# luisayang-malaxiangguo/Hybrid-GMRES

Hardware: AMD Instinct MI355X
Metric: GMRES iters/sec + SpMV GB/s (% HBM roofline), 2-D phantom A, 1/2/4/8 GPU (higher is better)
Workload: dtype f64

## Files before the change

hybrid-gmres_amd/csrc/capi.cpp:

```cpp
#include <limits.h>
#include <link.h>
#include <sched.h>

#include <chrono>
#include <cmath>
#include <cstdio>
#include <cstdlib>
#include <algorithm>
#include <cstring>
#include <set>
#include <vector>

#include "internal.h"

namespace hgm {

void DevBuf::ensure(size_t b) {
    if (b <= bytes) return;
    release();
    if (hipMalloc(&p, b) != hipSuccess) {
        p = nullptr;
        bytes = 0;
        throw Error{HGM_E_NOMEM, "hipMalloc failed for workspace (" + std::to_string(b) + " bytes)"};
    }
// ... 394 lines not shown

HGM_API void hgm_ctx_destroy(hgm_ctx* c) {
    if (!c) return;
    (void)hipSetDevice(c->device);
    if (c->stream) (void)hipStreamSynchronize(c->stream);
    if (c->host_stats)
        std::fprintf(stderr, "hgm host stats: %ld pipeline waits, %.3f ms blocked (%.2f us/wait)\n", c->waits,
                     c->wait_s * 1e3, c->waits ? c->wait_s * 1e6 / c->waits : 0.0);
    if (c->nccl) ncclCommDestroy(c->nccl);
    c->timing.clear();
    for (auto e : c->timing.pool) (void)hipEventDestroy(e);
    c->ws.clear();
    if (c->dscal) (void)hipFree(c->dscal);
    if (c->hscal) (void)hipHostFree(c->hscal);
    if (c->hstage) (void)hipHostFree(c->hstage);
    if (c->hup) (void)hipHostFree(c->hup);
    if (c->hring) (void)hipHostFree(c->hring);
    if (c->ev_pipe) (void)hipEventDestroy(c->ev_pipe);
    for (auto e : c->ev_step)
        if (e) (void)hipEventDestroy(e);
    if (c->aux) {
        (void)hipStreamSynchronize(c->aux);
        (void)hipStreamDestroy(c->aux);
    }
    if (c->stream) (void)hipStreamDestroy(c->stream);
    delete c;
}

HGM_API const char* hgm_last_error(const hgm_ctx* c) { return c ? c->err.c_str() : "null context"; }

HGM_API int hgm_ctx_set_option(hgm_ctx* c, int option, double v) {
    if (!c) return HGM_E_ARG;
    hgm::Numerics& n = c->num;
    const bool b01 = v == 0.0 || v == 1.0;
    auto bad = [&](const char* what) {
        c->err = std::string("hgm_ctx_set_option: ") + what;
        return HGM_E_ARG;
    };
    if (!HGM_EXPERIMENTS) {
        bool variant = false;
        switch (option) {
            case HGM_OPT_FUSED_REGION: variant = v != 64; break;
            case HGM_OPT_FUSED_BS: variant = v != 1024; break;
            case HGM_OPT_FUSED_DBG: variant = v != 0; break;
            case HGM_OPT_FUSED_PF: variant = v != 2; break;
            case HGM_OPT_FUSED_KIND: variant = v != 1; break;
            case HGM_OPT_FUSED_WAVES: variant = v != 4; break;
            case HGM_OPT_FUSED_GROUP: variant = v != 8; break;
            case HGM_OPT_FUSED_DEPTH: variant = v != 2; break;
            case HGM_OPT_FUSED_PAIRS: variant = v != 1; break;
            case HGM_OPT_FUSED_ACC32: variant = v != 1; break;
            case HGM_OPT_FUSED_REDUCE: variant = !(v == 0 || v == 1); break;
            case HGM_OPT_FUSED_ROWPAIR: variant = !(v == 0 || v == 4); break;
            default: break;
        }
        if (variant) return bad("a measured variant of the one-pass kernel: experiments build only (HGM_EXPERIMENTS=1)");
    }
    switch (option) {
        case HGM_OPT_PARITY: if (!b01) return bad("parity is 0 or 1"); n.parity = v != 0; break;
        case HGM_OPT_MGS_FORM: if (!b01) return bad("mgs form is 0 or 1"); n.mgs_form = (int)v; break;
        case HGM_OPT_MGS_SINGLE: if (!b01) return bad("mgs single is 0 or 1"); n.mgs_single = v != 0; break;
        case HGM_OPT_GRAM_ERR: if (!b01) return bad("gram err is 0 or 1"); n.gram_err = v != 0; break;
        case HGM_OPT_GRAM_ERR_MIN: if (!(v >= 0.0)) return bad("gram err min >= 0"); n.gram_err_min = v; break;
        case HGM_OPT_RING_POLL: if (!b01) return bad("ring poll is 0 or 1"); n.ring_poll = v != 0; break;
        case HGM_OPT_PEND_NORM:
            if (!(v == 0.0 || v == 1.0 || v == 2.0)) return bad("pend norm is 0, 1 or 2");
            n.pend_norm = (int)v;
            break;
        case HGM_OPT_RECON_SERIAL:
            if (v != -1.0 && !b01) return bad("recon serial is -1, 0 or 1");
            n.recon_serial = (int)v;
            break;
        case HGM_OPT_RECON_SERIAL_N: if (!(v >= 0.0)) return bad("recon serial n >= 0"); n.recon_serial_n = (int64_t)v; break;
        case HGM_OPT_PIPE_DEPTH:
            if (!(v >= 1.0 && v <= 6.0) || v != (double)(int)v) return bad("pipe depth is 1..6");
            n.pipe_depth = (int)v;
            break;
        case HGM_OPT_SYNC_EVENT_FENCE: if (!b01) return bad("sync event fence is 0 or 1"); n.sync_event_fence = v != 0; break;
        case HGM_OPT_MGS_PPL:
            if (!(v >= 1.0 && v <= 8.0) || v != (double)(int)v) return bad("mgs ppl is 1..8");
            n.mgs_ppl = (int)v;
            break;
        case HGM_OPT_MGS1_PPL:
            if (!(v == 0.0 || v == 1.0 || v == 2.0 || v == 4.0)) return bad("mgs1 ppl is 0, 1, 2 or 4");
            n.mgs1_ppl = (int)v;
            break;
        case HGM_OPT_MGS_FUSED: n.mgs_fused = v != 0.0; break;
        case HGM_OPT_LSQR_DEV: n.lsqr_dev = v != 0.0; break;
        case HGM_OPT_PAGED16: n.paged16 = v != 0.0; break;
        case HGM_OPT_BAND_DUAL: n.band_dual = v != 0.0; break;
        case HGM_OPT_FUSED_AB: if (!b01) return bad("fused_ab is 0 or 1"); n.fused_ab = v != 0; break;
        case HGM_OPT_FUSED_REGION:
            if (!(v >= 8 && v <= 1024 && v == std::floor(v))) return bad("fused_region is an integer in [8, 1024]");
            n.fused_region = (int)v;
            break;
        case HGM_OPT_FUSED_BS:
            if (!(v == 512 || v == 1024)) return bad("fused_bs is 512 or 1024");
            n.fused_bs = (int)v;
            break;
        case HGM_OPT_FUSED_PF: if (v < 0 || v > 4) return bad("fused_pf is 0..4"); n.fused_pf = v < 1 ? 1 : (int)v; break;
        case HGM_OPT_KRYLOV_PAD: if (v < -1 || v > 65536 || v != (double)(int64_t)v || (v > 0 && (int64_t)v % 64)) return bad("krylov_pad is -1 or a multiple of 64 in 0..65536"); n.krylov_pad = (int)v; break;
        case HGM_OPT_FUSED_DBG:
            if (!(v >= 0 && v <= 15 && v == std::floor(v))) return bad("fused_dbg is 0..15");
            n.fused_dbg = (int)v;
            break;
        case HGM_OPT_FUSED_KIND: if (!b01) return bad("fused_kind is 0 or 1"); n.fused_kind = (int)v; break;
        case HGM_OPT_FUSED_WREGION:
            if (!(v >= 4 && v <= 256 && v == std::floor(v))) return bad("fused_wregion is an integer in [4, 256]");
            n.fused_wregion = (int)v;
            break;
        case HGM_OPT_FUSED_WAVES:
            if (!(v == 1 || v == 2 || v == 4)) return bad("fused_waves is 1, 2 or 4");
            n.fused_waves = (int)v;
            break;
        case HGM_OPT_FUSED_GROUP:
            if (!(v == 4 || v == 8)) return bad("fused_group is 4 or 8");
            n.fused_group = (int)v;
            break;
        case HGM_OPT_FUSED_DEPTH:
            if (!(v == 2 || v == 3 || v == 4)) return bad("fused_depth is 2, 3 or 4");
            n.fused_depth = (int)v;
            break;
        case HGM_OPT_FUSED_PAIRS: if (!b01) return bad("fused_pairs is 0 or 1"); n.fused_pairs = v != 0; break;
        case HGM_OPT_FUSED_ACC32:
            if (!(v == 0 || v == 1 || v == 2)) return bad("fused_acc32 is 0, 1 or 2");
            n.fused_acc32 = (int)v;
            break;
        case HGM_OPT_FUSED_PLAN_DEV: if (!b01) return bad("fused_plan_dev is 0 or 1"); n.fused_plan_dev = v != 0; break;
        case HGM_OPT_FUSED_REDUCE:
            if (!(v == 0 || v == 1 || v == 2 || v == 3 || v == 4)) return bad("fused_reduce is 0 to 4");
            n.fused_reduce = (int)v;
            break;
        case HGM_OPT_FUSED_ROWPAIR:
            if (!(v == 0 || v == 1 || v == 2 || v == 3 || v == 4)) return bad("fused_rowpair is 0 to 4");
            n.fused_rowpair = (int)v;
            break;
        case HGM_OPT_FUSED_VSTREAM:
            if (!(v == 0 || v == 1 || v == 2 || v == 3)) return bad("fused_vstream is 0 to 3");
            n.fused_vstream = (int)v;
            break;
        case HGM_OPT_LSQR_RES_IMG: if (!b01) return bad("lsqr_res_img is 0 or 1"); n.lsqr_res_img = v != 0; break;
        case HGM_OPT_LSMR_FUSE_NMON: if (!b01) return bad("lsmr_fuse_nmon is 0 or 1"); n.lsmr_fuse_nmon = v != 0; break;
        case HGM_OPT_HOST_SPIN_US:
            if (!(v == std::floor(v) && std::fabs(v) <= 1e9)) return bad("host_spin_us is an integer");
            g_host_spin_us.store((int)v);
            break;
        default: return bad("unknown option");
    }
    return HGM_OK;
}

HGM_API int hgm_ctx_get_option(const hgm_ctx* c, int option, double* v) {
    if (!c || !v) return HGM_E_ARG;
    const hgm::Numerics& n = c->num;
    switch (option) {
        case HGM_OPT_PARITY: *v = n.parity; break;
        case HGM_OPT_MGS_FORM: *v = n.mgs_form; break;
        case HGM_OPT_MGS_SINGLE: *v = n.mgs_single; break;
        case HGM_OPT_GRAM_ERR: *v = n.gram_err; break;
        case HGM_OPT_GRAM_ERR_MIN: *v = n.gram_err_min; break;
        case HGM_OPT_RING_POLL: *v = n.ring_poll; break;
        case HGM_OPT_PEND_NORM: *v = n.pend_norm; break;
        case HGM_OPT_RECON_SERIAL: *v = n.recon_serial; break;
        case HGM_OPT_RECON_SERIAL_N: *v = (double)n.recon_serial_n; break;
        case HGM_OPT_PIPE_DEPTH: *v = n.pipe_depth; break;
        case HGM_OPT_SYNC_EVENT_FENCE: *v = n.sync_event_fence; break;
        case HGM_OPT_MGS_PPL: *v = n.mgs_ppl; break;
        case HGM_OPT_MGS1_PPL: *v = n.mgs1_ppl; break;
        case HGM_OPT_MGS_FUSED: *v = n.mgs_fused; break;
        case HGM_OPT_LSQR_DEV: *v = n.lsqr_dev; break;
        case HGM_OPT_PAGED16: *v = n.paged16; break;
        case HGM_OPT_BAND_DUAL: *v = n.band_dual; break;
        case HGM_OPT_FUSED_AB: *v = n.fused_ab; break;
        case HGM_OPT_FUSED_REGION: *v = n.fused_region; break;
        case HGM_OPT_FUSED_BS: *v = n.fused_bs; break;
        case HGM_OPT_FUSED_DBG: *v = n.fused_dbg; break;
        case HGM_OPT_FUSED_PF: *v = n.fused_pf; break;
        case HGM_OPT_KRYLOV_PAD: *v = n.krylov_pad; break;
        case HGM_OPT_FUSED_KIND: *v = n.fused_kind; break;
        case HGM_OPT_FUSED_WREGION: *v = n.fused_wregion; break;
        case HGM_OPT_FUSED_WAVES: *v = n.fused_waves; break;
        case HGM_OPT_FUSED_GROUP: *v = n.fused_group; break;
        case HGM_OPT_FUSED_DEPTH: *v = n.fused_depth; break;
        case HGM_OPT_FUSED_PAIRS: *v = n.fused_pairs; break;
        case HGM_OPT_FUSED_ACC32: *v = n.fused_acc32; break;
        case HGM_OPT_FUSED_PLAN_DEV: *v = n.fused_plan_dev; break;
        case HGM_OPT_FUSED_REDUCE: *v = n.fused_reduce; break;
        case HGM_OPT_FUSED_ROWPAIR: *v = n.fused_rowpair; break;
        case HGM_OPT_FUSED_VSTREAM: *v = n.fused_vstream; break;
        case HGM_OPT_LSQR_RES_IMG: *v = n.lsqr_res_img; break;
        case HGM_OPT_LSMR_FUSE_NMON: *v = n.lsmr_fuse_nmon; break;
        case HGM_OPT_HOST_SPIN_US: *v = g_host_spin_us.load(); break;
        default: return HGM_E_ARG;
    }
    return HGM_OK;
}

HGM_API int hgm_ctx_synchronize(hgm_ctx* c) {
    if (!c) return HGM_E_ARG;
    HGM_TRY(c, sync(c));
    return HGM_OK;
}

HGM_API void* hgm_ctx_stream(hgm_ctx* c) { return c ? (void*)c->stream : nullptr; }

HGM_API int hgm_ctx_rank(const hgm_ctx* c, int* rank, int* world) {
    if (!c) return HGM_E_ARG;
    if (rank) *rank = c->rank;
    if (world) *world = c->world;
    return HGM_OK;
}

HGM_API int hgm_ctx_release_workspace(hgm_ctx* c, int64_t* bytes_freed) {
    if (!c) return HGM_E_ARG;
    HGM_TRY(c, {
        HGM_HIP(hipSetDevice(c->device));
        HGM_HIP(hipStreamSynchronize(c->stream));
        if (c->aux) HGM_HIP(hipStreamSynchronize(c->aux));
        int64_t b = 0;
        for (auto& kv : c->ws) b += (int64_t)kv.second.bytes;
        c->ws.clear();
        if (bytes_freed) *bytes_freed = b;
    });
    return HGM_OK;
}

HGM_API int hgm_mem_info(hgm_ctx* c, int64_t* free_bytes, int64_t* total_bytes) {
    if (!c) return HGM_E_ARG;
    size_t f = 0, t = 0;
    if (hipSetDevice(c->device) != hipSuccess || hipMemGetInfo(&f, &t) != hipSuccess) return HGM_E_HIP;
    if (free_bytes) *free_bytes = (int64_t)f;
    if (total_bytes) *total_bytes = (int64_t)t;
    return HGM_OK;
}

HGM_API int hgm_ctx_solve_path(const hgm_ctx* c, int what, int* out, int cap, int* n) {
    if (!c || (what != 0 && what != 1) || cap < 0 || (cap > 0 && !out)) return HGM_E_ARG;
    std::vector<int> v;
    if (what == 0) v = c->path_mon;
    else if (c->path_onepass >= 0) v.push_back(c->path_onepass);
    for (int i = 0; i < cap && i < (int)v.size(); ++i) out[i] = v[i];
    if (n) *n = (int)v.size();
// ... 645 lines not shown
```

hybrid-gmres_amd/csrc/fused.hip:

```cpp
#include <algorithm>
#include <atomic>
#include <cstdio>
#include <cstdlib>
#include <cstring>
#include <chrono>
#include <numeric>
#include <thread>

#include "device_common.h"

namespace hgm {

namespace {
constexpr int FCH = 4096;
constexpr int FRMAX = 3968;
constexpr int FLRMAX = 768;
constexpr int FROWS = 128;
}
#ifndef HGM_FUSED_FGR
#define HGM_FUSED_FGR 16
#endif

struct FusedSub {
    int64_t e0;
// ... 717 lines not shown
                }
            } else {
                const int64_t e0 = readlane64(rpv, j), e1 = readlane64(rpv, j + 1);
                const int len = (int)(e1 - e0);
                b.len[j] = len;
                b.off[j] = 0;
                const __amdgpu_buffer_rsrc_t rv = buf_rsrc(val + e0, len * ES);
                const __amdgpu_buffer_rsrc_t rl = buf_rsrc(lidx + e0, len * 2);
#pragma unroll
                for (int c = 0; c < NCH; ++c) {
                    if constexpr (ES == 8)
                        b.v[j][c][0] = __builtin_bit_cast(double, __builtin_amdgcn_raw_buffer_load_b64(rv, (ln + CH * c) * 8, 0, 2));
                    else
                        b.v[j][c][0] = __builtin_bit_cast(float, __builtin_amdgcn_raw_buffer_load_b32(rv, (ln + CH * c) * 4, 0, 2));
                    b.s[j][c] = (uint32_t)__builtin_bit_cast(uint16_t, __builtin_amdgcn_raw_buffer_load_b16(rl, (ln + CH * c) * 2, 0, 2));
                }
            }
        }
    };
    T zx = T(0);
    const bool first_lane = (ln & (GL - 1)) == 0;
    (void)first_lane;
    auto process = [&](RB& b) {
        T P[G];
        uint32_t k[G][NCH][EPL];
        bool ia[RP ? G / 2 : 1][EPL];
        bool la_[RP == 2 ? G / 2 : 1];
        uint32_t kb[RP >= 3 ? G / 2 : 1][EPL];
        if constexpr (RP == 2) {
#pragma unroll
            for (int u = 0; u < G / 2; ++u) {
                const int offA = b.off[2 * u], offB = b.off[2 * u + 1];
                const int LA = (b.len[2 * u] + offA + 1) >> 1;
                const bool isA = ln < LA;
                la_[u] = isA;
                const int pos0 = isA ? 2 * ln - offA : 2 * (ln - LA) - offB;
                const int len = isA ? b.len[2 * u] : b.len[2 * u + 1];
                const uint32_t aoff = isA ? 0u : POFF;
                T p = T(0);
#pragma unroll
                for (int e = 0; e < EPL; ++e) {
                    const bool ok = (uint32_t)(pos0 + e) < (uint32_t)len;
                    const uint32_t sl = e ? b.s[u][0] >> 16 : b.s[u][0] & 0xffffu;
                    const uint32_t dm = (uint32_t)(MAXR - 64 + ln) * (uint32_t)ES;
                    const uint32_t kq = ok ? sl : dm;
                    p += b.v[u][0][e] * *reinterpret_cast<const T*>(reinterpret_cast<const char*>(qloc) + kq);
                    k[u][0][e] = ok ? sl * AS + aoff : dm * AS;
                }
                P[2 * u] = isA ? p : T(0);
                P[2 * u + 1] = isA ? T(0) : p;
            }
        } else if constexpr (VS) {
            const uint32_t dm = (uint32_t)(MAXR - 64 + ln) * (uint32_t)ES;
#pragma unroll
            for (int u = 0; u < G / 2; ++u) {
                const int la = b.len[2 * u];
                const uint32_t s = b.off[2 * u] ? b.s[u][0] : (dm | (dm << 16) | 0xc007c007u);
                T pa = T(0), pb = T(0);
#pragma unroll
                for (int e = 0; e < EPL; ++e) {
                    const bool inA = 2 * ln + e < la;
                    const uint32_t sl = (e ? s >> 16 : s) & 0x3ff8u;
                    const uint32_t c8 = (e ? __builtin_amdgcn_alignbit(s, s, 27) : s >> 11) & 0xf8u;
                    const T v = b.v[u][0][e] + *reinterpret_cast<const T*>(reinterpret_cast<const char*>(qloc) + VTAB * ES + c8);
                    b.v[u][0][e] = v;
                    const uint32_t ka = inA ? sl : dm, kk = inA ? dm : sl;
                    const T qa = *reinterpret_cast<const T*>(reinterpret_cast<const char*>(qloc) + ka);
                    const T qb = *reinterpret_cast<const T*>(reinterpret_cast<const char*>(qloc) + kk);
                    if constexpr (HGM_FUSED_FMA) {
                        pa = fma_t(v, qa, pa);
                        pb = fma_t(v, qb, pb);
                    } else {
                        pa = pa + v * qa;
                        pb = pb + v * qb;
                    }
                    k[u][0][e] = ka;
                    kb[u][e] = kk;
                }
                P[2 * u] = pa;
                P[2 * u + 1] = pb;
            }
        } else if constexpr (RP == 1 || RP >= 3) {
#pragma unroll
            for (int u = 0; u < G / 2; ++u) {
                const int la = b.len[2 * u], lab = la + b.len[2 * u + 1];
                T pa = T(0), pb = T(0);
#pragma unroll
                for (int e = 0; e < EPL; ++e) {
                    const int pos = EPL * ln - b.off[2 * u] + e;
                    const bool inA = (uint32_t)pos < (uint32_t)la;
                    const bool in = (uint32_t)pos < (uint32_t)lab;
                    const uint32_t sl = e ? b.s[u][0] >> 16 : b.s[u][0] & 0xffffu;
                    const uint32_t dm = (uint32_t)(MAXR - 64 + ln) * (uint32_t)ES;
                    if constexpr (RP == 4) {
                        const uint32_t ka = inA ? sl : dm, kk = (in && !inA) ? sl : dm;
                        const T qa = *reinterpret_cast<const T*>(reinterpret_cast<const char*>(qloc) + ka);
                        const T qb = *reinterpret_cast<const T*>(reinterpret_cast<const char*>(qloc) + kk);
                        if constexpr (HGM_FUSED_FMA) {
                            pa = fma_t(b.v[u][0][e], qa, pa);
                            pb = fma_t(b.v[u][0][e], qb, pb);
                        } else {
                            pa = pa + b.v[u][0][e] * qa;
                            pb = pb + b.v[u][0][e] * qb;
                        }
                        k[u][0][e] = ka * AS;
                        kb[u][e] = kk * AS;
                        ia[u][e] = inA;
                        continue;
                    }
                    const uint32_t kq = in ? sl : dm;
                    const T p = b.v[u][0][e] * *reinterpret_cast<const T*>(reinterpret_cast<const char*>(qloc) + kq);
                    pa = pa + (inA ? p : T(0));
                    pb = pb + (inA ? T(0) : p);
                    if constexpr (RP == 3) {
                        k[u][0][e] = inA ? sl * AS : dm * AS;
                        kb[u][e] = (in && !inA) ? sl * AS : dm * AS;
                    } else {
                        k[u][0][e] = in ? sl * AS + (inA ? 0u : POFF) : dm * AS;
                    }
                    ia[u][e] = inA;
                }
                P[2 * u] = pa;
                P[2 * u + 1] = pb;
            }
        }
#pragma unroll
        for (int j = 0; j < G && !RP; ++j) {
            T p = T(0);
#pragma unroll
            for (int c = 0; c < NCH; ++c)
// ... 77 lines not shown
                    TA* pa = reinterpret_cast<TA*>(reinterpret_cast<char*>(ac) + k[u][0][e]);
                    if constexpr (AM == 2) {
                        lds_add(pa, (double)b.v[u][0][e] * (double)sj);
                    } else if constexpr (AM == 1) {
                        const T t = b.v[u][0][e] * sj;
                        *pa = *pa + t;
                    } else {
                        lds_add(pa, b.v[u][0][e] * sj);
                    }
                }
            }
        }
#pragma unroll
        for (int j = 0; j < G && !RP; ++j) {
            const T sj = lane_bcast(zs, j * GL);
#pragma unroll
            for (int c = 0; c < NCH; ++c)
#pragma unroll
                for (int e = 0; e < EPL; ++e) {
                    TA* pa = reinterpret_cast<TA*>(reinterpret_cast<char*>(ac) + k[j][c][e] * AS);
                    if constexpr (DBG & 2) {
                        S += b.v[j][c][e] * sj;
                    } else if constexpr (AM == 2) {
                        lds_add(pa, (double)b.v[j][c][e] * (double)sj);
                    } else if constexpr (AM == 1) {
                        const T t = b.v[j][c][e] * sj;
                        *pa = *pa + t;
                    } else {
                        lds_add(pa, b.v[j][c][e] * sj);
                    }
                }
        }
    };
    RB b[D];
    int a[D], cn[D], un[D];
    int64_t r[D];
#pragma unroll
    for (int i = 0; i < D; ++i) {
        next(a[i], cn[i], un[i]);
        r[i] = load_rp(a[i], cn[i], un[i]);
    }
    stage();
#pragma unroll
    for (int i = 0; i < D - 1; ++i) issue(b[i], a[i], cn[i], r[i], un[i]);
    __syncthreads();
    do {
#pragma unroll
        for (int t = 0; t < D; ++t) {
            const int ti = (t + D - 1) % D;
            next(a[t], cn[t], un[t]);
            r[t] = load_rp(a[t], cn[t], un[t]);
            issue(b[ti], a[ti], cn[ti], r[ti], un[ti]);
            __builtin_amdgcn_sched_barrier(0);
            process(b[t]);
            __builtin_amdgcn_sched_barrier(0);
        }
    } while (b[0].cnt > 0);
    if (zx_part) zx = wave_sum(zx);
    __syncthreads();
    if (zx_part && ln == 0) qloc[wv] = zx;
    for (int k = threadIdx.x; k < nr; k += 64 * W) {
        TA t = acc[0][0][k];
        if constexpr (NA == 2) t += acc[0][1][k];
#pragma unroll
        for (int w = 1; w < W; ++w) {
            t += acc[w][0][k];
            if constexpr (NA == 2) t += acc[w][1][k];
        }
        if constexpr (HGM_PART_NT) __builtin_nontemporal_store(t, &part[pb + k]);
        else part[pb + k] = t;
    }
    if (zx_part) {
        __syncthreads();
        if (threadIdx.x == 0) {
            T t = qloc[0];
#pragma unroll
            for (int w = 1; w < W; ++w) t += qloc[w];
            zx_part[g] = t;
        }
    }
}

namespace {
template <typename F>
void parallel_for(int64_t n, F f) {
    unsigned nt = std::thread::hardware_concurrency();
    nt = std::max(1u, std::min(nt, 16u));
    if (n < 64 || nt == 1) {
        for (int64_t i = 0; i < n; ++i) f(i);
        return;
    }
    std::vector<std::thread> th;
    const int64_t step = (n + nt - 1) / nt;
    for (unsigned t = 0; t < nt; ++t) {
        const int64_t a = t * step, b = std::min<int64_t>(n, a + step);
        if (a >= b) break;
        th.emplace_back([=, &f]() {
            for (int64_t i = a; i < b; ++i) f(i);
        });
    }
    for (auto& t : th) t.join();
}

template <typename T>
T* upload(const std::vector<T>& v) {
    T* d = nullptr;
    const size_t bytes = std::max<size_t>(v.size(), 1) * sizeof(T);
// ... 734 lines not shown
        int64_t done = 0;
        for (const int2& r : rr[g]) {
            for (int s = r.x; s < r.x + r.y; ++s) {
                while (w < W - 1 && done * W >= tot * (w + 1)) ++w;
                auto& v = wr[(size_t)g * W + w];
                if (!v.empty() && v.back().x + v.back().y == s) ++v.back().y;
                else v.push_back(make_int2(s, 1));
                done += rp[s + 1] - rp[s];
            }
        }
    });
    const int rpmode = c->num.fused_rowpair;
    bool rowpair = rpmode && c->num.fused_pairs && W == 4 && G == 8 && c->num.fused_depth == 2 &&
                         c->num.fused_dbg == 0 &&
                   (es == 8 || c->num.fused_acc32 == 1 || (c->num.fused_acc32 == 2 && rpmode == 4)) &&
                   maxlen + 1 <= 128;
    auto fits = [&](int64_t s) {
        if (rpmode != 2) return (rp[s + 2] - rp[s]) + (rp[s] & 1) <= 128;
        const int64_t la = rp[s + 1] - rp[s] + (rp[s] & 1), lb = rp[s + 2] - rp[s + 1] + (rp[s + 1] & 1);
        return (la + 1) / 2 + (lb + 1) / 2 <= 64;
    };
    if (rowpair) {
        std::vector<std::vector<int2>> wr1(wr.size());
        std::atomic<bool> over{false};
        parallel_for((int64_t)wr.size(), [&](int64_t i) {
            std::vector<int2>& out = wr1[(size_t)i];
            for (const int2& r : wr[(size_t)i]) {
                int s0 = r.x;
                const int end = r.x + r.y;
                int s = r.x;
                while (s < end) {
                    if (s + 1 < end && !fits(s)) {
                        out.push_back(make_int2(s0, s + 1 - s0));
                        s0 = s + 1;
                        s = s + 1;
                    } else {
                        s += 2;
                    }
                }
                if (s0 < end) out.push_back(make_int2(s0, end - s0));
            }
            if (out.size() > 64) over = true;
        });
        if (over) rowpair = false;
        else wr.swap(wr1);
    }
    std::vector<int32_t> wrun((size_t)nreg * W + 1, 0);
    for (size_t i = 0; i < wr.size(); ++i) {
        HGM_REQUIRE(wr[i].size() <= 64, "fused A*(B*q): more than 64 row runs per wave");
        wrun[i + 1] = wrun[i] + (int32_t)wr[i].size();
    }
    std::vector<int2> runs(std::max<int32_t>(wrun.back(), 1));
    for (size_t i = 0; i < wr.size(); ++i) std::copy(wr[i].begin(), wr[i].end(), runs.begin() + wrun[i]);
    if (dev_build) return fused_plan_dev_finish(c, B, R, W, G, rowpair ? rpmode : 0, es, nreg, maxlen, wrun, runs, t0);
    std::vector<std::vector<int32_t>> rrays(nreg);
    std::vector<uint16_t> lidx(std::max<int64_t>(nnz, 1) + 256, 0);
    std::atomic<int> worst{0};
    {
        unsigned nt = std::max(1u, std::min(std::thread::hardware_concurrency(), 16u));
        std::vector<std::thread> th;
        std::atomic<int64_t> nextg{0};
        for (unsigned t = 0; t < nt; ++t)
            th.emplace_back([&]() {
                std::vector<int32_t> map(m, -1);
                for (int64_t g; (g = nextg.fetch_add(1)) < nreg;) {
                    auto& rs = rrays[g];
                    for (const int2& r : rr[g])
                        for (int64_t e = rp[r.x]; e < rp[r.x + r.y]; ++e) rs.push_back(ci[e]);
                    std::sort(rs.begin(), rs.end());
                    rs.erase(std::unique(rs.begin(), rs.end()), rs.end());
                    int cur = worst.load();
                    while ((int)rs.size() > cur && !worst.compare_exchange_weak(cur, (int)rs.size())) {}
                    if (rs.size() > (size_t)RW_SLOTS_MAX - 64) continue;
                    for (size_t k = 0; k < rs.size(); ++k) map[rs[k]] = (int32_t)k;
                    for (const int2& r : rr[g])
                        for (int64_t e = rp[r.x]; e < rp[r.x + r.y]; ++e) lidx[e] = (uint16_t)(map[ci[e]] * es);
                    for (int32_t ray : rs) map[ray] = -1;
                }
            });
        for (auto& t : th) t.join();
    }
    int maxr = 0;
#define HGM_RW_PICK(WV, MRV) \
    if (W == WV && worst.load() <= MRV - 64 && (maxr == 0 || MRV < maxr)) maxr = MRV;
    HGM_RW_SHAPES(HGM_RW_PICK)
#undef HGM_RW_PICK
    HGM_REQUIRE(maxr > 0, kLdsCapacityMsg);
    std::vector<int64_t> reg_base(nreg + 1, 0);
    for (int64_t g = 0; g < nreg; ++g) reg_base[g + 1] = reg_base[g] + (int64_t)rrays[g].size();
    const int64_t nslot = reg_base[nreg];
    HGM_REQUIRE(nslot < (int64_t(1) << 31), "fused A*(B*q): partial slots");
    std::vector<int32_t> ray_tab(std::max<int64_t>(nslot, 1));
    for (int64_t g = 0; g < nreg; ++g) std::copy(rrays[g].begin(), rrays[g].end(), ray_tab.begin() + reg_base[g]);
    std::vector<int64_t> rs_ptr(m + 1, 0);
    for (int64_t g = 0; g < nreg; ++g)
        for (int32_t ray : rrays[g]) rs_ptr[ray + 1]++;
    for (int64_t i = 0; i < m; ++i) rs_ptr[i + 1] += rs_ptr[i];
    std::vector<int32_t> rs_slot(std::max<int64_t>(nslot, 1));
    {
        std::vector<int64_t> fill(rs_ptr.begin(), rs_ptr.end() - 1);
        for (int64_t g = 0; g < nreg; ++g)
            for (size_t r = 0; r < rrays[g].size(); ++r) rs_slot[fill[rrays[g][r]]++] = (int32_t)(reg_base[g] + r);
    }
    FusedPlan* P = new FusedPlan;
    try {
        P->kind = 1;
// ... 67 lines not shown
    hgm_mat* Bm = const_cast<hgm_mat*>(B);
    const Numerics& nu = c->num;
    const bool rw = nu.fused_kind == 1;
    const int64_t key = fused_key(nu);
    if (Bm->fused && Bm->fused_key != key) {
        fused_plan_free(Bm->fused);
        Bm->fused = nullptr;
    }
    if (!Bm->fused && Bm->fused_failed_key != key) {
        try {
            if (rw) {
                for (int R = nu.fused_wregion;; R /= 2) {
                    try {
                        Bm->fused = fused_plan_build_rw(c, B, R, nu.fused_waves, nu.fused_group);
                        break;
                    } catch (const Error& e) {
                        if (e.code != HGM_E_ARG || e.msg != kLdsCapacityMsg || R / 2 < 16 || R % 2) throw;
                    }
                }
            } else {
                Bm->fused = fused_plan_build(c, B, nu.fused_region);
            }
            Bm->fused_key = key;
            Bm->fused_failed_key = -1;
        } catch (const Error& e) {
            if (e.code != HGM_E_ARG) throw;
            Bm->fused_failed_key = key;
        }
    }
    return Bm->fused;
}

#define HGM_RW_SHAPES_GK(X) X(4, 1088) X(4, 1344) X(4, 1536) X(4, 2048)
template <typename T, bool GK>
static bool fused_rw_launch(hgm_ctx* c, const hgm_mat* B, const FusedPlan* P, const FusedArgs<T>& fa, bool dry) {
    const int W = P->waves, MR = P->maxr, G = P->group, D = c->num.fused_depth;
    const bool PRm = c->num.fused_pairs;
    const int64_t ml = P->maxlen + (PRm ? 1 : 0);
    const int NC = ml <= (PRm ? 128 : 64) ? 1 : ml <= (PRm ? 256 : 128) ? 2 : 4;
    const int dbg = c->num.fused_dbg;
    const int am = sizeof(T) == 4 ? c->num.fused_acc32 : 0;
    const bool side = fa.side_out != nullptr && (fa.xt != nullptr || fa.side_sq);
#define HGM_RWL(AMV, WV, MRV, GV, NCV, DV, PV, DBV) HGM_RWLR(AMV, WV, MRV, GV, NCV, DV, PV, DBV, 0)
#define HGM_RWLR(AMV, WV, MRV, GV, NCV, DV, PV, DBV, RPV)                                                            \
    {                                                                                                                 \
        if (!dry)                                                                                                     \
            launch(c, false, k_fused_rw<T, GK, AMV, WV, MRV, GV, NCV, DV, PV, DBV, RPV>, dim3((unsigned)P->nreg),   \
                   dim3(64 * WV), (const int64_t*)P->reg_base, (const int32_t*)P->ray_tab, (const int32_t*)P->wrun, \
                   (const int2*)P->runs, (const int64_t*)B->rp, (const T*)B->val, (const uint16_t*)P->lidx, fa.q,  \
                   fa.zraw, (typename AccT<T, AMV>::t*)P->part, side ? fa.xt : nullptr,                            \
                   side ? (T*)P->zx_part : nullptr, fa.ev, fa.easq, fa.zout, fa.side_sq ? 1 : 0, fa.pn, VStream{}); \
        return true;                                                                                                  \
    }
#define HGM_RWLV(MRV)                                                                                                \
    {                                                                                                                 \
        if (!dry)                                                                                                     \
            launch(c, false, k_fused_rw<T, GK, 0, 4, MRV, 8, 1, 2, true, 0, 5>, dim3((unsigned)P->nreg), dim3(256), \
                   (const int64_t*)P->reg_base, (const int32_t*)P->ray_tab, (const int32_t*)P->wrun,                \
                   (const int2*)P->runs, (const int64_t*)nullptr, (const T*)P->vs_vals,                             \
                   (const uint16_t*)P->vs_slots, fa.q, fa.zraw, (T*)P->part, side ? fa.xt : nullptr,                \
                   side ? (T*)P->zx_part : nullptr, fa.ev, fa.easq, fa.zout, fa.side_sq ? 1 : 0, fa.pn,             \
                   VStream{P->vs_desc, P->vs_run_unit, P->vs_table});                                                \
        return true;                                                                                                  \
    }
    if (P->rowpair) {
        constexpr int AMP = sizeof(T) == 4 ? 1 : 0;
#if HGM_EXPERIMENTS
        if constexpr (sizeof(T) == 4)
            if (am == 2 && P->rowpair == 4 && !dbg && W == 4 && G == 8 && NC == 1 && PRm && D == 2 && MR == 2048)
                HGM_RWLR(2, 4, 2048, 8, 1, 2, true, 0, 4)
#endif
        if (dbg || W != 4 || G != 8 || NC != 1 || !PRm || D != 2 || am != AMP) {
            if (dry) return false;
            throw Error{HGM_E_ARG, "fused A*(B*q): row pairs take 4 waves, 8 rows, one chunk, pairs, depth 2, "
                                   "the production accumulation"};
        }
        if constexpr (sizeof(T) == 8 && !GK) {
            if (P->rowpair == 4 && P->vs_on) {
                if (MR == 1088) HGM_RWLV(1088)
                if (MR == 1344) HGM_RWLV(1344)
                if (MR == 1536) HGM_RWLV(1536)
                if (MR == 2048) HGM_RWLV(2048)
            }
        }
        if (P->rowpair == 4) {
            if (MR == 1088) HGM_RWLR(AMP, 4, 1088, 8, 1, 2, true, 0, 4)
            if (MR == 1344) HGM_RWLR(AMP, 4, 1344, 8, 1, 2, true, 0, 4)
            if (MR == 1536) HGM_RWLR(AMP, 4, 1536, 8, 1, 2, true, 0, 4)
            if (MR == 2048) HGM_RWLR(AMP, 4, 2048, 8, 1, 2, true, 0, 4)
        }
#if HGM_EXPERIMENTS
        if (P->rowpair == 3 && MR == 2048) HGM_RWLR(AMP, 4, 2048, 8, 1, 2, true, 0, 3)
        if (P->rowpair == 1 && MR == 2048) HGM_RWLR(AMP, 4, 2048, 8, 1, 2, true, 0, 1)
        if (P->rowpair == 2 && MR == 2048) HGM_RWLR(AMP, 4, 2048, 8, 1, 2, true, 0, 2)
#endif
        if (dry) return false;
        throw Error{HGM_E_ARG, "fused A*(B*q): no row-pair kernel for this plan's shape and the options"};
    }
    if constexpr (GK) {
        constexpr int AMP = sizeof(T) == 4 ? 1 : 0;
        const bool dshape = W == 4 && MR == 2048 && G == 8 && NC == 1 && PRm && D == 2;
        if (dbg) {
#if HGM_EXPERIMENTS
            if (dshape && am == AMP) {
#define HGM_RWD(DV) if (dbg == DV) HGM_RWL(AMP, 4, 2048, 8, 1, 2, true, DV)
                HGM_RWD(1) HGM_RWD(2) HGM_RWD(4) HGM_RWD(7)
#undef HGM_RWD
            }
#endif
            if (dry) return false;
            throw Error{HGM_E_ARG, "fused_dbg (Golub-Kahan / fp32 pass): waves 4, 2048 slots, 8 rows, pairs, depth 2, one chunk; 1, 2, 4 or 7"};
        }
#if HGM_EXPERIMENTS
        if constexpr (sizeof(T) == 4) {
            if (dshape && am == 0) HGM_RWL(0, 4, 2048, 8, 1, 2, true, 0)
            if (dshape && am == 2) HGM_RWL(2, 4, 2048, 8, 1, 2, true, 0)
        }
#endif
        (void)dshape;
        if (am == AMP) {
#define HGM_RW(WV, MRV)                                                                                              \
    if (W == WV && MR == MRV && G == 8 && PRm && D == 2) {                                                           \
        if (NC == 1) HGM_RWL(AMP, WV, MRV, 8, 1, 2, true, 0)                                                        \
        if (NC == 2) HGM_RWL(AMP, WV, MRV, 8, 2, 2, true, 0)                                                        \
    }
            HGM_RW_SHAPES_GK(HGM_RW)
#undef HGM_RW
        }
    } else {
        if (dbg) {
#if HGM_EXPERIMENTS
            if (W == 4 && MR == 2048 && G == 8 && NC == 1 && PRm && D == 2) {
#define HGM_RWD(DV) if (dbg == DV) HGM_RWL(0, 4, 2048, 8, 1, 2, true, DV)
                HGM_RWD(1) HGM_RWD(2) HGM_RWD(3) HGM_RWD(4) HGM_RWD(5) HGM_RWD(6) HGM_RWD(7)
#undef HGM_RWD
// ... 213 lines not shown
```

hybrid-gmres_amd/csrc/internal.h:

```cpp
#pragma once

#include <hip/hip_runtime.h>
#include <rccl/rccl.h>

#include <atomic>
#include <chrono>
#include <cstdint>
#include <map>
#include <string>
#include <utility>
#include <vector>

#include "hgmres.h"

#ifndef HGM_EXPERIMENTS
#define HGM_EXPERIMENTS 0
#endif

namespace hgm {

struct Error {
    int code;
    std::string msg;
};

#define HGM_HIP(expr)                                                                   \
    do {                                                                                \
        hipError_t e_ = (expr);                                                         \
        if (e_ != hipSuccess)                                                           \
            throw ::hgm::Error{HGM_E_HIP, std::string(#expr) + ": " + hipGetErrorString(e_)}; \
    } while (0)

#define HGM_REQUIRE(cond, msg)                                \
    do {                                                      \
        if (!(cond)) throw ::hgm::Error{HGM_E_ARG, (msg)};    \
    } while (0)

constexpr int BS = 256;
constexpr int MAX_PARTS = 1024;
constexpr int NSCAL = 512;

struct DevBuf {
    void* p = nullptr;
    size_t bytes = 0;
    void ensure(size_t b);
    void release();
    ~DevBuf() { release(); }
};

enum KClass { KC_SPMV_A = 0, KC_SPMV_B = 1, KC_MGS = 2, KC_FUSED = 3, KC_PNORM = 4, KC_SPMM = 5, KC_N = 6 };

struct Timing {
    bool on = false;
    bool paused = false;
    unsigned mask = 0xffu;
    std::vector<std::pair<hipEvent_t, hipEvent_t>> ev[KC_N];
    double bytes[KC_N] = {0, 0, 0, 0, 0, 0};
    std::vector<hipEvent_t> pool;
    hipEvent_t get();
    void clear();
};

struct Numerics {
    bool parity = false;
    int mgs_form = 1;
    bool mgs_single = true;
    bool gram_err = true;
    double gram_err_min = 0.01;
    bool ring_poll = true;
    int pend_norm = 1;
    int recon_serial = -1;
    int64_t recon_serial_n = int64_t(4) << 20;
    int pipe_depth = 2;
    bool sync_event_fence = false;
    int mgs_ppl = 1;
    int mgs1_ppl = 0;
    bool mgs_fused = true;
    bool lsqr_dev = true;
    bool paged16 = true;
    bool band_dual = true;
    bool fused_ab = true;
    int fused_region = 64;
    int fused_bs = 1024;
    int fused_pf = 2;
    int fused_kind = 1;
    int fused_wregion = 32;
    int fused_waves = 4;
    int fused_group = 8;
    int fused_depth = 2;
    bool fused_pairs = true;
    int fused_acc32 = 1;
    bool fused_plan_dev = true;
    int fused_rowpair = 4;
    int fused_vstream = 1;
    int fused_reduce = 0;
    bool lsqr_res_img = true;
    bool lsmr_fuse_nmon = true;
    int krylov_pad = -1;
    int fused_dbg = 0;
};
struct FusedPlan;

}

struct hgm_ctx {
    hgm::Numerics num;
    int device = 0;
    hipStream_t stream = nullptr;
    int rank = 0, world = 1;
    ncclComm_t nccl = nullptr;
    hgm_allreduce_fn host_ar = nullptr;
    void* host_ar_user = nullptr;
    std::string err;
    std::map<std::string, hgm::DevBuf> ws;
    double* dscal = nullptr;
    double* hscal = nullptr;
    double* hstage = nullptr;
    size_t hstage_bytes = 0;
    double* hup = nullptr;
    size_t hup_bytes = 0;
    double* hring = nullptr;
    double* hring_dev = nullptr;
    size_t hring_bytes = 0;
    hipEvent_t ev_pipe = nullptr;
    hipStream_t aux = nullptr;
    hipEvent_t ev_step[8] = {};
    unsigned ev_flags[9] = {};
    std::string ws_tag;
    bool host_stats = false;
    double wait_s = 0.0;
    long waits = 0;
    hipEvent_t arm_start = nullptr, arm_stop = nullptr, cur_stop = nullptr;
    hgm::Timing timing;
    std::vector<int> path_mon;
    int path_onepass = -1;

    template <typename T>
    T* buf(const std::string& name, size_t count) {
        auto& b = ws_tag.empty() ? ws[name] : ws[ws_tag + name];
        b.ensure(count * sizeof(T) + 256);
        return reinterpret_cast<T*>(b.p);
    }
};

namespace hgm {
struct PixOrder {
    int N = 0, tile = 1, super = 0;
// ... 425 lines not shown
```

hybrid-gmres_amd/hgmres/_lib.py:

```python
from __future__ import annotations

import ctypes as C
import os

_HERE = os.path.dirname(os.path.abspath(__file__))
LIB_PATH = os.environ.get("HGM_LIB") or os.path.join(_HERE, "libhgmres.so")

HGM_OK = 0
HGM_E_ARG = -1
HGM_E_HIP = -2
HGM_E_NOMEM = -3
HGM_E_COMM = -4
HGM_E_NOT_ASSIGNED = -5
HGM_E_UNSUPPORTED = -6

HGM_F64, HGM_F32 = 0, 1
OPTIONS = {"parity": 1, "mgs_form": 2, "mgs_single": 3, "gram_err": 4, "gram_err_min": 5, "ring_poll": 6,
           "pend_norm": 7, "recon_serial": 8, "recon_serial_n": 9, "pipe_depth": 10, "sync_event_fence": 11,
           "mgs_ppl": 12, "mgs1_ppl": 13, "mgs_fused": 14, "lsqr_dev": 15, "paged16": 16,
           "band_dual": 17, "fused_ab": 18, "fused_region": 19, "fused_bs": 20, "fused_dbg": 21, "fused_pf": 22,
           "krylov_pad": 23, "fused_kind": 24, "fused_wregion": 25, "fused_waves": 26, "fused_group": 27,
           "fused_depth": 28, "fused_pairs": 29, "fused_acc32": 30, "fused_plan_dev": 31, "fused_reduce": 32,
           "host_spin_us": 33, "fused_rowpair": 34,
           "lsqr_res_img": 35, "lsmr_fuse_nmon": 36}
OPTIONS_37 = {"fused_vstream": 37}


def option_id(name):
    return OPTIONS[name] if name in OPTIONS else OPTIONS_37[name]

HGM_MGS, HGM_CGS2 = 0, 1
HGM_SIDE_AB, HGM_SIDE_BA = 0, 1
HGM_DEVICE_PTRS = 1
HGM_EXPLICIT_RESIDUAL = 2
HGM_UNIQUE_ID_BYTES = 128

c_int, c_int64, c_double, c_void_p = C.c_int, C.c_int64, C.c_double, C.c_void_p
P = C.POINTER
dp = P(c_double)
ip64 = P(c_int64)
ip32 = P(C.c_int32)

ALLREDUCE_FN = C.CFUNCTYPE(c_int, dp, c_int64, c_void_p)


class hgm_opts(C.Structure):
    _fields_ = [("flags", c_int), ("orth", c_int), ("H_out", dp)]


_SIGS = {
    "hgm_version": (c_int, []),
    "hgm_runtime_check": (c_int, [C.c_char_p, c_int]),
    "hgm_ctx_set_option": (c_int, [c_void_p, c_int, c_double]),
    "hgm_ctx_get_option": (c_int, [c_void_p, c_int, P(c_double)]),
    "hgm_device_count": (c_int, [P(c_int)]),
    "hgm_ctx_create": (c_int, [c_int, P(c_void_p)]),
    "hgm_comm_unique_id": (c_int, [c_void_p]),
    "hgm_ctx_create_dist": (c_int, [c_int, c_int, c_int, c_void_p, P(c_void_p)]),
    "hgm_ctx_set_host_allreduce": (c_int, [c_void_p, c_int, c_int, ALLREDUCE_FN, c_void_p]),
    "hgm_ctx_destroy": (None, [c_void_p]),
    "hgm_last_error": (C.c_char_p, [c_void_p]),
    "hgm_ctx_synchronize": (c_int, [c_void_p]),
    "hgm_ctx_stream": (c_void_p, [c_void_p]),
    "hgm_ctx_rank": (c_int, [c_void_p, P(c_int), P(c_int)]),
    "hgm_experiments": (c_int, []),
    "hgm_ctx_release_workspace": (c_int, [c_void_p, P(c_int64)]),
    "hgm_mem_info": (c_int, [c_void_p, P(c_int64), P(c_int64)]),
    "hgm_ctx_solve_path": (c_int, [c_void_p, c_int, P(c_int), c_int, P(c_int)]),
    "hgm_mat_create_csr": (c_int, [c_void_p, c_int64, c_int64, c_int64, ip64, ip32, dp, c_int, P(c_void_p)]),
    "hgm_mat_create_csr_tiled": (c_int, [c_void_p, c_int64, c_int64, c_int64, ip64, ip32, dp, c_int, c_int, c_int, c_int,
                                         P(c_void_p)]),
    "hgm_mat_create_csc": (c_int, [c_void_p, c_int64, c_int64, c_int64, ip64, ip64, dp, c_int, P(c_void_p)]),
    "hgm_mat_transpose": (c_int, [c_void_p, c_void_p, P(c_void_p)]),
    "hgm_mat_create_siddon": (c_int, [c_void_p, c_int, c_int, c_double, c_int, P(c_void_p)]),
    "hgm_mat_create_siddon_ordered": (c_int, [c_void_p, c_int, c_int, c_double, c_int, c_int, c_int,
                                              P(c_void_p)]),
    "hgm_mat_create_fanbeam": (c_int, [c_void_p, c_int, c_int, c_double, c_double, c_double, c_int, c_int, c_int,
                                       P(c_void_p)]),
# ... 88 lines not shown
```

include/hgmres.h:

```cpp
#ifndef HGMRES_H
#define HGMRES_H

#include <stdint.h>

#ifdef __cplusplus
extern "C" {
#endif

#define HGM_API __attribute__((visibility("default")))

#define HGM_VERSION 100
#define HGM_UNIQUE_ID_BYTES 128

typedef struct hgm_ctx hgm_ctx;
typedef struct hgm_mat hgm_mat;

enum hgm_status {
    HGM_OK = 0,
    HGM_E_ARG = -1,
    HGM_E_HIP = -2,
    HGM_E_NOMEM = -3,
    HGM_E_COMM = -4,
    HGM_E_NOT_ASSIGNED = -5,
    HGM_E_UNSUPPORTED = -6
// ... 1 lines not shown

enum hgm_dtype { HGM_F64 = 0, HGM_F32 = 1 };
enum hgm_orth { HGM_MGS = 0, HGM_CGS2 = 1 };
enum hgm_side { HGM_SIDE_AB = 0, HGM_SIDE_BA = 1 };

enum hgm_flags {
    HGM_DEVICE_PTRS = 1,
    HGM_EXPLICIT_RESIDUAL = 2
};

typedef struct hgm_opts {
    int flags;
    int orth;
    double* H_out;
} hgm_opts;

enum hgm_ctx_option {
    HGM_OPT_PARITY = 1,
    HGM_OPT_MGS_FORM = 2,
    HGM_OPT_MGS_SINGLE = 3,
    HGM_OPT_GRAM_ERR = 4,
    HGM_OPT_GRAM_ERR_MIN = 5,
    HGM_OPT_RING_POLL = 6,
    HGM_OPT_PEND_NORM = 7,
    HGM_OPT_RECON_SERIAL = 8,
    HGM_OPT_RECON_SERIAL_N = 9,
    HGM_OPT_PIPE_DEPTH = 10,
    HGM_OPT_SYNC_EVENT_FENCE = 11,
    HGM_OPT_MGS_PPL = 12,
    HGM_OPT_MGS1_PPL = 13,
    HGM_OPT_MGS_FUSED = 14,
    HGM_OPT_LSQR_DEV = 15,
    HGM_OPT_PAGED16 = 16,
    HGM_OPT_BAND_DUAL = 17,
    HGM_OPT_FUSED_AB = 18,
    HGM_OPT_FUSED_REGION = 19,
    HGM_OPT_FUSED_BS = 20,
    HGM_OPT_FUSED_DBG = 21,
    HGM_OPT_FUSED_PF = 22,
    HGM_OPT_KRYLOV_PAD = 23        ,
    HGM_OPT_FUSED_KIND = 24,
    HGM_OPT_FUSED_WREGION = 25,
    HGM_OPT_FUSED_WAVES = 26,
    HGM_OPT_FUSED_GROUP = 27,
    HGM_OPT_FUSED_DEPTH = 28,
    HGM_OPT_FUSED_PAIRS = 29,
    HGM_OPT_FUSED_ACC32 = 30       ,
    HGM_OPT_FUSED_PLAN_DEV = 31,
    HGM_OPT_FUSED_REDUCE = 32,
    HGM_OPT_HOST_SPIN_US = 33      ,
    HGM_OPT_FUSED_ROWPAIR = 34     ,
    HGM_OPT_LSQR_RES_IMG = 35      ,
    HGM_OPT_LSMR_FUSE_NMON = 36    ,
    HGM_OPT_FUSED_VSTREAM = 37
};

typedef int (*hgm_allreduce_fn)(double* buf, int64_t count, void* user);

HGM_API int hgm_version(void);
HGM_API int hgm_experiments(void);
HGM_API int hgm_runtime_check(char* msg, int len);
HGM_API int hgm_device_count(int* count);
HGM_API int hgm_ctx_create(int device, hgm_ctx** ctx);
HGM_API int hgm_comm_unique_id(void* id_out );
HGM_API int hgm_ctx_create_dist(int device, int rank, int world, const void* unique_id, hgm_ctx** ctx);
HGM_API int hgm_ctx_set_host_allreduce(hgm_ctx* ctx, int rank, int world, hgm_allreduce_fn fn, void* user);
HGM_API void hgm_ctx_destroy(hgm_ctx* ctx);
HGM_API const char* hgm_last_error(const hgm_ctx* ctx);
HGM_API int hgm_ctx_synchronize(hgm_ctx* ctx);
HGM_API void* hgm_ctx_stream(hgm_ctx* ctx);
HGM_API int hgm_ctx_rank(const hgm_ctx* ctx, int* rank, int* world);
HGM_API int hgm_ctx_release_workspace(hgm_ctx* ctx, int64_t* bytes_freed);
HGM_API int hgm_mem_info(hgm_ctx* ctx, int64_t* free_bytes, int64_t* total_bytes);
HGM_API int hgm_ctx_solve_path(const hgm_ctx* ctx, int what, int* out, int cap, int* n);
HGM_API int hgm_ctx_set_option(hgm_ctx* ctx, int option, double value);
HGM_API int hgm_ctx_get_option(const hgm_ctx* ctx, int option, double* value);

HGM_API int hgm_mat_create_csr(hgm_ctx* ctx, int64_t rows, int64_t cols, int64_t nnz,
                               const int64_t* row_ptr, const int32_t* col_idx,
                               const double* val, int dtype, hgm_mat** out);
HGM_API int hgm_mat_create_csr_tiled(hgm_ctx* ctx, int64_t rows, int64_t cols, int64_t nnz, const int64_t* row_ptr,
                                     const int32_t* col_idx, const double* val, int dtype, int N, int tile,
                                     int super_block, hgm_mat** out);
HGM_API int hgm_mat_create_csc(hgm_ctx* ctx, int64_t rows, int64_t cols, int64_t nnz,
                               const int64_t* jc, const int64_t* ir, const double* pr,
                               int dtype, hgm_mat** out);
HGM_API int hgm_mat_transpose(hgm_ctx* ctx, const hgm_mat* in, hgm_mat** out);
HGM_API int hgm_mat_row_slice(hgm_ctx* ctx, const hgm_mat* in, int64_t lo, int64_t hi, hgm_mat** out);
HGM_API int hgm_mat_create_siddon(hgm_ctx* ctx, int N, int n_angles, double det_offset,
                                  int dtype, hgm_mat** out);
HGM_API int hgm_mat_create_siddon_ordered(hgm_ctx* ctx, int N, int n_angles, double det_offset,
                                          int dtype, int tile, int super_block, hgm_mat** out);
HGM_API int hgm_mat_create_fanbeam(hgm_ctx* ctx, int N, int n_angles, double R, double span, double det_offset,
                                   int dtype, int tile, int super_block, hgm_mat** out);
HGM_API int hgm_mat_create_backprojector(hgm_ctx* ctx, int N, int n_angles, double det_offset, int dtype,
                                         int tile, int super_block, hgm_mat** out);
HGM_API int hgm_mat_order(const hgm_mat* mat, int which, int* N, int* tile, int* super_block);
HGM_API int hgm_mat_info(const hgm_mat* mat, int64_t* rows, int64_t* cols, int64_t* nnz, int* dtype);
HGM_API int hgm_mat_tune(hgm_mat* mat, int variant, int group);
HGM_API int hgm_mat_set_bands(hgm_ctx* ctx, hgm_mat* mat, int64_t band_width, int group);
HGM_API int hgm_mat_download(hgm_ctx* ctx, const hgm_mat* mat, int64_t* row_ptr, int32_t* col_idx, double* val);
HGM_API void hgm_mat_destroy(hgm_mat* mat);

HGM_API int hgm_spmv(hgm_ctx* ctx, const hgm_mat* A, const void* x_dev, void* y_dev);

HGM_API int hgm_spmv_ab(hgm_ctx* ctx, const hgm_mat* A, const hgm_mat* B, const void* q_dev, void* Bq_dev,
                        void* ABq_dev);
// ... 108 lines not shown
```

Measured before the change: 499.0.

## Batch LDS gathers in compact-stream kernel and deepen its batch ring to three

Measured after the change: 505.4, median of 6. 1.3% higher.

```diff
diff --git a/hybrid-gmres_amd/csrc/capi.cpp b/hybrid-gmres_amd/csrc/capi.cpp
--- a/hybrid-gmres_amd/csrc/capi.cpp
+++ b/hybrid-gmres_amd/csrc/capi.cpp
@@ -470,6 +470,7 @@
             case HGM_OPT_FUSED_ACC32: variant = v != 1; break;
             case HGM_OPT_FUSED_REDUCE: variant = !(v == 0 || v == 1); break;
             case HGM_OPT_FUSED_ROWPAIR: variant = !(v == 0 || v == 4); break;
+            case HGM_OPT_FUSED_VSDEPTH: variant = (v == 2 || v == 3 || v == 4) && !(v == 2 || v == HGM_VSDEPTH_DEFAULT); break;
             default: break;
         }
         if (variant) return bad("a measured variant of the one-pass kernel: experiments build only (HGM_EXPERIMENTS=1)");
@@ -556,6 +557,10 @@
         case HGM_OPT_FUSED_VSTREAM:
             if (!(v == 0 || v == 1 || v == 2 || v == 3)) return bad("fused_vstream is 0 to 3");
             n.fused_vstream = (int)v;
+            break;
+        case HGM_OPT_FUSED_VSDEPTH:
+            if (!(v == 2 || v == 3 || v == 4)) return bad("fused_vsdepth is 2, 3 or 4");
+            n.fused_vsdepth = (int)v;
             break;
         case HGM_OPT_LSQR_RES_IMG: if (!b01) return bad("lsqr_res_img is 0 or 1"); n.lsqr_res_img = v != 0; break;
         case HGM_OPT_LSMR_FUSE_NMON: if (!b01) return bad("lsmr_fuse_nmon is 0 or 1"); n.lsmr_fuse_nmon = v != 0; break;
@@ -606,6 +611,7 @@
         case HGM_OPT_FUSED_REDUCE: *v = n.fused_reduce; break;
         case HGM_OPT_FUSED_ROWPAIR: *v = n.fused_rowpair; break;
         case HGM_OPT_FUSED_VSTREAM: *v = n.fused_vstream; break;
+        case HGM_OPT_FUSED_VSDEPTH: *v = n.fused_vsdepth; break;
         case HGM_OPT_LSQR_RES_IMG: *v = n.lsqr_res_img; break;
         case HGM_OPT_LSMR_FUSE_NMON: *v = n.lsmr_fuse_nmon; break;
         case HGM_OPT_HOST_SPIN_US: *v = g_host_spin_us.load(); break;
diff --git a/hybrid-gmres_amd/csrc/fused.hip b/hybrid-gmres_amd/csrc/fused.hip
--- a/hybrid-gmres_amd/csrc/fused.hip
+++ b/hybrid-gmres_amd/csrc/fused.hip
@@ -793,30 +793,56 @@
             }
         } else if constexpr (VS) {
             const uint32_t dm = (uint32_t)(MAXR - 64 + ln) * (uint32_t)ES;
+            uint32_t c8[G / 2][EPL];
 #pragma unroll
             for (int u = 0; u < G / 2; ++u) {
                 const int la = b.len[2 * u];
                 const uint32_t s = b.off[2 * u] ? b.s[u][0] : (dm | (dm << 16) | 0xc007c007u);
-                T pa = T(0), pb = T(0);
 #pragma unroll
                 for (int e = 0; e < EPL; ++e) {
                     const bool inA = 2 * ln + e < la;
                     const uint32_t sl = (e ? s >> 16 : s) & 0x3ff8u;
-                    const uint32_t c8 = (e ? __builtin_amdgcn_alignbit(s, s, 27) : s >> 11) & 0xf8u;
-                    const T v = b.v[u][0][e] + *reinterpret_cast<const T*>(reinterpret_cast<const char*>(qloc) + VTAB * ES + c8);
-                    b.v[u][0][e] = v;
-                    const uint32_t ka = inA ? sl : dm, kk = inA ? dm : sl;
-                    const T qa = *reinterpret_cast<const T*>(reinterpret_cast<const char*>(qloc) + ka);
-                    const T qb = *reinterpret_cast<const T*>(reinterpret_cast<const char*>(qloc) + kk);
+                    c8[u][e] = (e ? __builtin_amdgcn_alignbit(s, s, 27) : s >> 11) & 0xf8u;
+                    k[u][0][e] = inA ? sl : dm;
+                    kb[u][e] = inA ? dm : sl;
+                    asm volatile("" : "+v"(c8[u][e]), "+v"(k[u][0][e]), "+v"(kb[u][e]));
+                }
+            }
+            __builtin_amdgcn_sched_barrier(0);
+            T tb[G / 2][EPL], qa[G / 2][EPL], qb[G / 2][EPL];
+#pragma unroll
+            for (int u = 0; u < G / 2; ++u)
+#pragma unroll
+                for (int e = 0; e < EPL; ++e)
+                    tb[u][e] = *reinterpret_cast<const T*>(reinterpret_cast<const char*>(qloc) + VTAB * ES + c8[u][e]);
+#pragma unroll
+            for (int u = 0; u < G / 2; ++u)
+#pragma unroll
+                for (int e = 0; e < EPL; ++e) {
+                    qa[u][e] = *reinterpret_cast<const T*>(reinterpret_cast<const char*>(qloc) + k[u][0][e]);
+                    qb[u][e] = *reinterpret_cast<const T*>(reinterpret_cast<const char*>(qloc) + kb[u][e]);
+                }
+            __builtin_amdgcn_sched_barrier(0);
+#pragma unroll
+            for (int u = 0; u < G / 2; ++u) {
+                asm volatile("" : "+v"(tb[u][0]), "+v"(tb[u][EPL - 1]));
+#pragma unroll
+                for (int e = 0; e < EPL; ++e) b.v[u][0][e] = b.v[u][0][e] + tb[u][e];
+            }
+#pragma unroll
+            for (int u = 0; u < G / 2; ++u) {
+                asm volatile("" : "+v"(qa[u][0]), "+v"(qb[u][0]), "+v"(qa[u][EPL - 1]), "+v"(qb[u][EPL - 1]));
+                T pa = T(0), pb = T(0);
+#pragma unroll
+                for (int e = 0; e < EPL; ++e) {
+                    const T v = b.v[u][0][e];
                     if constexpr (HGM_FUSED_FMA) {
-                        pa = fma_t(v, qa, pa);
-                        pb = fma_t(v, qb, pb);
+                        pa = fma_t(v, qa[u][e], pa);
+                        pb = fma_t(v, qb[u][e], pb);
                     } else {
-                        pa = pa + v * qa;
-                        pb = pb + v * qb;
+                        pa = pa + v * qa[u][e];
+                        pb = pb + v * qb[u][e];
                     }
-                    k[u][0][e] = ka;
-                    kb[u][e] = kk;
                 }
                 P[2 * u] = pa;
                 P[2 * u + 1] = pb;
@@ -1000,7 +1026,7 @@
             r[t] = load_rp(a[t], cn[t], un[t]);
             issue(b[ti], a[ti], cn[ti], r[ti], un[ti]);
             __builtin_amdgcn_sched_barrier(0);
-            process(b[t]);
+            if (!VS || b[t].cnt > 0) process(b[t]);
             __builtin_amdgcn_sched_barrier(0);
         }
     } while (b[0].cnt > 0);
@@ -1841,6 +1867,17 @@
     }
     std::vector<int2> runs(std::max<int32_t>(wrun.back(), 1));
     for (size_t i = 0; i < wr.size(); ++i) std::copy(wr[i].begin(), wr[i].end(), runs.begin() + wrun[i]);
+    if (std::getenv("HGM_FUSED_VERBOSE")) {
+        int64_t nb = 0, empty[5] = {0, 0, 0, 0, 0};
+        for (size_t w = 0; w + 1 < wrun.size(); ++w) {
+            int64_t b = 0;
+            for (int i = wrun[w]; i < wrun[w + 1]; ++i) b += (runs[i].y + G - 1) / G;
+            nb += b;
+            for (int D = 2; D <= 4; ++D) empty[D] += std::max<int64_t>(1, (b + D - 1) / D) * D - b;
+        }
+        std::fprintf(stderr, "[fused rw plan] %lld waves, %lld batches; empty batches at ring depth 2: %lld, 3: %lld, 4: %lld\n",
+                     (long long)wrun.size() - 1, (long long)nb, (long long)empty[2], (long long)empty[3], (long long)empty[4]);
+    }
     if (dev_build) return fused_plan_dev_finish(c, B, R, W, G, rowpair ? rpmode : 0, es, nreg, maxlen, wrun, runs, t0);
     std::vector<std::vector<int32_t>> rrays(nreg);
     std::vector<uint16_t> lidx(std::max<int64_t>(nnz, 1) + 256, 0);
@@ -2014,10 +2051,10 @@
                    side ? (T*)P->zx_part : nullptr, fa.ev, fa.easq, fa.zout, fa.side_sq ? 1 : 0, fa.pn, VStream{}); \
         return true;                                                                                                  \
     }
-#define HGM_RWLV(MRV)                                                                                                \
+#define HGM_RWLV(MRV, DV)                                                                                            \
     {                                                                                                                 \
         if (!dry)                                                                                                     \
-            launch(c, false, k_fused_rw<T, GK, 0, 4, MRV, 8, 1, 2, true, 0, 5>, dim3((unsigned)P->nreg), dim3(256), \
+            launch(c, false, k_fused_rw<T, GK, 0, 4, MRV, 8, 1, DV, true, 0, 5>, dim3((unsigned)P->nreg), dim3(256), \
                    (const int64_t*)P->reg_base, (const int32_t*)P->ray_tab, (const int32_t*)P->wrun,                \
                    (const int2*)P->runs, (const int64_t*)nullptr, (const T*)P->vs_vals,                             \
                    (const uint16_t*)P->vs_slots, fa.q, fa.zraw, (T*)P->part, side ? fa.xt : nullptr,                \
@@ -2039,10 +2076,24 @@
         }
         if constexpr (sizeof(T) == 8 && !GK) {
             if (P->rowpair == 4 && P->vs_on) {
-                if (MR == 1088) HGM_RWLV(1088)
-                if (MR == 1344) HGM_RWLV(1344)
-                if (MR == 1536) HGM_RWLV(1536)
-                if (MR == 2048) HGM_RWLV(2048)
+                const int VD = c->num.fused_vsdepth;
+#define HGM_RWLVD(DV)                                                                                                \
+    if (VD == DV) {                                                                                                   \
+        if (MR == 1088) HGM_RWLV(1088, DV)                                                                            \
+        if (MR == 1344) HGM_RWLV(1344, DV)                                                                            \
+        if (MR == 1536) HGM_RWLV(1536, DV)                                                                            \
+        if (MR == 2048) HGM_RWLV(2048, DV)                                                                            \
+    }
+                HGM_RWLVD(2)
+#if HGM_EXPERIMENTS || HGM_VSDEPTH_DEFAULT == 3
+                HGM_RWLVD(3)
+#endif
+#if HGM_EXPERIMENTS || HGM_VSDEPTH_DEFAULT == 4
+                HGM_RWLVD(4)
+#endif
+#undef HGM_RWLVD
+                if (dry) return false;
+                throw Error{HGM_E_ARG, "fused A*(B*q): no compact-stream kernel for this plan's shape and fused_vsdepth"};
             }
         }
         if (P->rowpair == 4) {
diff --git a/hybrid-gmres_amd/csrc/internal.h b/hybrid-gmres_amd/csrc/internal.h
--- a/hybrid-gmres_amd/csrc/internal.h
+++ b/hybrid-gmres_amd/csrc/internal.h
@@ -15,6 +15,9 @@
 
 #ifndef HGM_EXPERIMENTS
 #define HGM_EXPERIMENTS 0
+#endif
+#ifndef HGM_VSDEPTH_DEFAULT
+#define HGM_VSDEPTH_DEFAULT 3
 #endif
 
 namespace hgm {
@@ -93,6 +96,7 @@
     bool fused_plan_dev = true;
     int fused_rowpair = 4;
     int fused_vstream = 1;
+    int fused_vsdepth = HGM_VSDEPTH_DEFAULT;
     int fused_reduce = 0;
     bool lsqr_res_img = true;
     bool lsmr_fuse_nmon = true;
diff --git a/hybrid-gmres_amd/hgmres/_lib.py b/hybrid-gmres_amd/hgmres/_lib.py
--- a/hybrid-gmres_amd/hgmres/_lib.py
+++ b/hybrid-gmres_amd/hgmres/_lib.py
@@ -23,7 +23,7 @@
            "fused_depth": 28, "fused_pairs": 29, "fused_acc32": 30, "fused_plan_dev": 31, "fused_reduce": 32,
            "host_spin_us": 33, "fused_rowpair": 34,
            "lsqr_res_img": 35, "lsmr_fuse_nmon": 36}
-OPTIONS_37 = {"fused_vstream": 37}
+OPTIONS_37 = {"fused_vstream": 37, "fused_vsdepth": 38}
 
 
 def option_id(name):
diff --git a/include/hgmres.h b/include/hgmres.h
--- a/include/hgmres.h
+++ b/include/hgmres.h
@@ -77,7 +77,8 @@
     HGM_OPT_FUSED_ROWPAIR = 34     ,
     HGM_OPT_LSQR_RES_IMG = 35      ,
     HGM_OPT_LSMR_FUSE_NMON = 36    ,
-    HGM_OPT_FUSED_VSTREAM = 37
+    HGM_OPT_FUSED_VSTREAM = 37     ,
+    HGM_OPT_FUSED_VSDEPTH = 38
 };
 
 typedef int (*hgm_allreduce_fn)(double* buf, int64_t count, void* user);
```
